# shanjiayao/PTT

Measured on AMD Instinct MI355X. Metric: tracklet frames/sec (hot path: PointNet++ SA stack + Point-Track-Transformer blocks), higher is better.
Workload: dtype f32

## Files before the change

include/ptt_hip.h:

```cpp
#ifndef PTT_HIP_H
#define PTT_HIP_H

#include <stddef.h>
#include <stdint.h>

#ifdef __cplusplus
extern "C" {
#endif

#define PTT_ABI_VERSION 34

enum {
    PTT_OK = 0,
    PTT_EINVAL = -1,
    PTT_EUNSUPPORTED = -2,
    PTT_ELAUNCH = -3,
    PTT_EWORKSPACE = -4
};

typedef void* ptt_stream_t;

int ptt_version(void);
const char* ptt_error_name(int code);
const char* ptt_last_error_string(void);

int ptt_fps_f32(const float* xyz, int B, int N, int npoint, int32_t* idx_out,
                ptt_stream_t stream);
int ptt_fps_ws_f32(const float* xyz, int B, int N, int npoint, int32_t* idx_out, float* workspace,
                   size_t workspace_elems, ptt_stream_t stream);

int ptt_ffps_f32(const float* xyz, const float* feat, int64_t feat_sb, int64_t feat_sc, int64_t feat_sn,
                 int B, int N, int C, int npoint, int32_t* idx_out, ptt_stream_t stream);

int ptt_gather_f32(const float* feat, const int32_t* idx, int B, int C, int N, int M,
                   float* out, ptt_stream_t stream);
int ptt_gather_grad_f32(const float* grad_out, const int32_t* idx, int B, int C, int N,
                        int M, float* grad_feat, ptt_stream_t stream);

int ptt_select_centres_f32(const float* xyz, const int32_t* idx, int B, int N, int M, float* new_xyz,
                           int64_t* idx64_out, ptt_stream_t stream);

int ptt_ball_query_f32(const float* new_xyz, const float* xyz, int B, int M, int N,
                       float radius, int nsample, int32_t* idx_out, ptt_stream_t stream);

int ptt_centres_ball_query_f32(const float* xyz, const int32_t* sel, int B, int N, int M, float radius, int nsample,
                               float* new_xyz, int64_t* idx64_out, int32_t* idx_out, ptt_stream_t stream);

int ptt_group_f32(const float* feat, const int32_t* idx, int B, int C, int N, int M,
                  int ns, float* out, ptt_stream_t stream);
int ptt_group_grad_f32(const float* grad_out, const int32_t* idx, int B, int C, int N,
                       int M, int ns, float* grad_feat, ptt_stream_t stream);

size_t ptt_scatter_add_det_workspace(int B, int N, int E);
int ptt_scatter_add_det_f32(const float* src, const int32_t* idx, int B, int C, int N, int E, float* out,
                            void* workspace, size_t workspace_bytes, ptt_stream_t stream);

int ptt_knn_f32(const float* xyz, int B, int N, int k, int32_t* idx_out,
                ptt_stream_t stream);
int ptt_knn_rel_f32(const float* xyz, int B, int N, int k, int32_t* idx_out, float* rel_out,
                    ptt_stream_t stream);

size_t ptt_packed_weight_elems(int Cout, int K);
// ... 523 lines not shown
```

ptt_amd/csrc/point_ops.hip:

```cpp
#pragma clang fp contract(off)

#include <limits.h>
#include <stdlib.h>
#include "common.h"

namespace ptt {

__device__ __forceinline__ float sqdist3(float ax, float ay, float az, float bx, float by, float bz) {
    const float dx = ax - bx, dy = ay - by, dz = az - bz;
    return (dx * dx + dy * dy) + dz * dz;
}

__device__ __forceinline__ float knn_dist(float ax, float ay, float az, float bx, float by, float bz) {
    const float d = sqdist3(ax, ay, az, bx, by, bz);
    return d < __builtin_inff() ? d : 3.402823466e+38f;
}

__device__ __forceinline__ float lane_bcast(float v, int src_lane) {
    return __builtin_bit_cast(float, __builtin_amdgcn_readlane(__builtin_bit_cast(int, v), src_lane));
}

typedef float fps_f2 __attribute__((ext_vector_type(2)));


// ... 160 lines not shown
            } else if constexpr (LX) {
                lx = xyz_lds[3 * gi + 0]; ly = xyz_lds[3 * gi + 1]; lz = xyz_lds[3 * gi + 2];
            } else {
                if (gd < 0.f) { gx = pts[0]; gy = pts[1]; gz = pts[2]; }
                lx = gx; ly = gy; lz = gz;
            }
            if (t == 0) sel_lds[j] = gi;
        }
    }
    __syncthreads();
    for (int j = t; j < npoint; j += T) out[j] = sel_lds[j];
}

template <int T, int P>
static int launch_fps(const float* xyz, int B, int N, int npoint, int32_t* idx, hipStream_t s) {
    const size_t sel_bytes = (size_t)((npoint + 3) & ~3) * sizeof(int);
    if (sel_bytes + (size_t)N * 12 + 1024 <= 65536 && !dev_switches().fps_plain) {
#ifdef PTT_DEV
        if (const char* e = getenv("PTT_FPS_ABL")) {
            const int abl = atoi(e);
#define PTT_FPS_ABL_CASE(A) if (abl == A) { hipLaunchKernelGGL((fps_kernel<T, P, true, A>), dim3(B), dim3(T), sel_bytes + (size_t)N * 12, s, xyz, N, npoint, idx); return check_launch("fps_kernel(abl)"); }
            PTT_FPS_ABL_CASE(1) PTT_FPS_ABL_CASE(2) PTT_FPS_ABL_CASE(3) PTT_FPS_ABL_CASE(4) PTT_FPS_ABL_CASE(8) PTT_FPS_ABL_CASE(12) PTT_FPS_ABL_CASE(15)
            PTT_FPS_ABL_CASE(16) PTT_FPS_ABL_CASE(32) PTT_FPS_ABL_CASE(47) PTT_FPS_ABL_CASE(7) PTT_FPS_ABL_CASE(24) PTT_FPS_ABL_CASE(40)
#undef PTT_FPS_ABL_CASE
        }
#endif
        hipLaunchKernelGGL((fps_kernel<T, P, true>), dim3(B), dim3(T), sel_bytes + (size_t)N * 12, s, xyz, N, npoint, idx);
        return check_launch("fps_kernel");
    }
    hipLaunchKernelGGL((fps_kernel<T, P, false>), dim3(B), dim3(T), sel_bytes, s, xyz, N, npoint, idx);
    return check_launch("fps_kernel");
}

template <int CPW>
__device__ __forceinline__ void ball_sweep(const float* __restrict__ pts, int N, float r2, int ns, const float (&cx)[CPW],
                                           const float (&cy)[CPW], const float (&cz)[CPW], int ncentres,
                                           int32_t* __restrict__ out0, int lane) {
    int cnt[CPW], first[CPW];
#pragma unroll
    for (int c = 0; c < CPW; ++c) { cnt[c] = (c < ncentres) ? 0 : ns; first[c] = 0; }
    for (int base = 0; base < N; base += 64) {
        const int k = base + lane;
        const bool in = k < N;
        float px = 0.f, py = 0.f, pz = 0.f;
        if (in) { px = pts[3 * k + 0]; py = pts[3 * k + 1]; pz = pts[3 * k + 2]; }
        bool active = false;
#pragma unroll
        for (int c = 0; c < CPW; ++c) {
            if (cnt[c] >= ns) continue;
            const float d = sqdist3(cx[c], cy[c], cz[c], px, py, pz);
            const bool hit = in && d < r2;
            const unsigned long long mask = __ballot(hit);
            if (mask != 0ull) {
                if (cnt[c] == 0) first[c] = base + (__ffsll((long long)mask) - 1);
                const int pos = cnt[c] + __popcll(mask & ((1ull << lane) - 1ull));
                if (hit && pos < ns) out0[(size_t)c * ns + pos] = k;
                cnt[c] += __popcll(mask);
            }
            active = active || cnt[c] < ns;
        }
        if (!active) break;
    }
#pragma unroll
    for (int c = 0; c < CPW; ++c) {
        if (c >= ncentres) break;
        const int fill = (cnt[c] > 0) ? first[c] : 0;
// ... 908 lines not shown
    if (N <= 64) return launch_fps<64, 1>(xyz, B, N, npoint, idx_out, s);
    if (N <= 128) return launch_fps<64, 2>(xyz, B, N, npoint, idx_out, s);
    if (N <= 256) return launch_fps<64, 4>(xyz, B, N, npoint, idx_out, s);
    if (N <= 512) {
        if (const int T = dev_switches().fps_t) {
            if (T == 256) return launch_fps<256, 2>(xyz, B, N, npoint, idx_out, s);
            if (T == 128) return launch_fps<128, 4>(xyz, B, N, npoint, idx_out, s);
            if (T == 512) return launch_fps<512, 1>(xyz, B, N, npoint, idx_out, s);
        }
        return launch_fps<64, 8>(xyz, B, N, npoint, idx_out, s);
    }
    if (N <= 1024) {
        if (const int T = dev_switches().fps_t) {
            if (T == 64) return launch_fps<64, 16>(xyz, B, N, npoint, idx_out, s);
            if (T == 128) return launch_fps<128, 8>(xyz, B, N, npoint, idx_out, s);
            if (T == 512) return launch_fps<512, 2>(xyz, B, N, npoint, idx_out, s);
        }
        return launch_fps<256, 4>(xyz, B, N, npoint, idx_out, s);
    }
    if (N <= 2048) {
        if (const int T = dev_switches().fps_t) {
            if (T == 512) return launch_fps<512, 4>(xyz, B, N, npoint, idx_out, s);
            if (T == 1024) return launch_fps<1024, 2>(xyz, B, N, npoint, idx_out, s);
            if (T == 128) return launch_fps<128, 16>(xyz, B, N, npoint, idx_out, s);
        }
        return launch_fps<256, 8>(xyz, B, N, npoint, idx_out, s);
    }
    if (N <= 4096) return launch_fps<512, 8>(xyz, B, N, npoint, idx_out, s);
    if (N <= 8192) return launch_fps<1024, 8>(xyz, B, N, npoint, idx_out, s);
    if (N <= 16384) return launch_fps<1024, 16>(xyz, B, N, npoint, idx_out, s);
    return fail(PTT_EUNSUPPORTED, "ptt_fps_f32: N=%d exceeds the register-resident limit 16384 (use ptt_fps_ws_f32)", N);
}

extern "C" int ptt_spatial_order_f32(const float* xyz, int B, int N, int32_t* order, ptt_stream_t stream) {
    if (B < 0 || N <= 0) return fail(PTT_EINVAL, "ptt_spatial_order_f32: B=%d N=%d", B, N);
    if (B == 0) return PTT_OK;
    if (!xyz || !order) return fail(PTT_EINVAL, "ptt_spatial_order_f32: null pointer");
    if (N > 8192 || (long long)B * N > INT_MAX) return fail(PTT_EUNSUPPORTED, "ptt_spatial_order_f32: N=%d (at most 8192 points per cloud are sorted in LDS)", N);
    int P = 2;
    while (P < N) P <<= 1;
    const int lds = P * (int)sizeof(unsigned long long);
    return launch("spatial_order_kernel", spatial_order_kernel, dim3(B), dim3(1024), lds, as_stream(stream), xyz, N, P, order);
}

extern "C" int ptt_fps_ws_f32(const float* xyz, int B, int N, int npoint, int32_t* idx_out, float* workspace, size_t workspace_elems,
                              ptt_stream_t stream) {
    if (B < 0 || N <= 0 || npoint < 0) return fail(PTT_EINVAL, "ptt_fps_ws_f32: B=%d N=%d npoint=%d", B, N, npoint);
    if (B == 0 || npoint == 0) return PTT_OK;
    if (!xyz || !idx_out) return fail(PTT_EINVAL, "ptt_fps_ws_f32: null pointer");
    if ((long long)N * 3 > INT_MAX) return fail(PTT_EUNSUPPORTED, "ptt_fps_ws_f32: N=%d", N);
    if (!workspace || workspace_elems < (size_t)B * N)
        return fail(PTT_EWORKSPACE, "ptt_fps_ws_f32: %zu floats of workspace needed", (size_t)B * N);
    hipLaunchKernelGGL(fps_ws_kernel, dim3(B), dim3(1024), 0, as_stream(stream), xyz, N, npoint, workspace, idx_out);
    return check_launch("fps_ws_kernel");
}

extern "C" int ptt_ffps_f32(const float* xyz, const float* feat, int64_t feat_sb, int64_t feat_sc, int64_t feat_sn, int B, int N, int C,
                            int npoint, int32_t* idx_out, ptt_stream_t stream) {
    if (B < 1 || N < 1 || npoint < 1 || C < 0) return fail(PTT_EINVAL, "ptt_ffps_f32: B=%d N=%d C=%d npoint=%d", B, N, C, npoint);
    if (!xyz || !idx_out || (C > 0 && !feat)) return fail(PTT_EINVAL, "ptt_ffps_f32: null pointer");
    if (N > FFPS_MAX_N || C > FFPS_MAX_C || npoint > FFPS_MAX_NPOINT)
        return fail(PTT_EUNSUPPORTED, "ptt_ffps_f32: N=%d C=%d npoint=%d exceed the limits N <= %d, C <= %d, npoint <= %d", N, C, npoint,
                    FFPS_MAX_N, FFPS_MAX_C, FFPS_MAX_NPOINT);
    if (C > 0 && (long long)(N - 1) * llabs((long long)feat_sn) + (long long)(C - 1) * llabs((long long)feat_sc) > INT_MAX)
        return fail(PTT_EUNSUPPORTED, "ptt_ffps_f32: one cloud's features span more than 2^31 elements (strides %lld, %lld)",
                    (long long)feat_sc, (long long)feat_sn);
// ... 292 lines not shown
```

ptt_amd/models/backbones_3d/pointnet2/pointnet2_modules.py:

```python
import os
from typing import List

import torch
import torch.nn as nn
import torch.nn.functional as F

from .... import ops, train_ops
from ....param_cache import (DropsCachesOnModeChange, FoldedLayer, ParamCache, conv_bn_tensors, fold_conv_bn,
                             index_table)
from . import pointnet2_utils
from . import pytorch_utils as pt_utils

STREAM_COMPACT_MIN_BALLS = 2048
STREAM_COMPACT_MAX_POINTS = 1024


class PointnetSAModuleVotes(DropsCachesOnModeChange, nn.Module):
    def __init__(self, *, mlp: List[int], radius: float = None, nsample: int = None, bn: bool = True,
                 use_xyz: bool = True, normalize_xyz: bool = False, sample_uniformly: bool = False,
                 sample_method='fps'):
        super().__init__()
        self.radius = radius
        self.nsample = nsample
        self.mlp_module = None
        self.use_xyz = use_xyz
        self.normalize_xyz = normalize_xyz
        self.sample_uniformly = sample_uniformly
        self.grouper = pointnet2_utils.QueryAndGroup(radius, nsample, use_xyz=use_xyz, ret_grouped_xyz=True,
                                                     normalize_xyz=normalize_xyz, sample_uniformly=sample_uniformly,
                                                     ret_unique_cnt=False)
        mlp_spec = mlp
        if use_xyz and len(mlp_spec) > 0:
            mlp_spec[0] += 3
        self.mlp_module = pt_utils.SharedMLP(mlp_spec, bn=bn)
        self.sample_method = sample_method
        self._fused_cache = ParamCache()
        self.centres_knn_k = 0
        self.centres_knn = None

    def _sample(self, xyz, features, npoint):
        if self.sample_method == 'fps':
            return pointnet2_utils.furthest_point_sample(xyz, npoint)
        if self.sample_method in ('rs', 'sequence'):
            return index_table(xyz.size(0), npoint, xyz.device, torch.int32)
        if self.sample_method == 'ffps':
            if features is None:
                raise ValueError("sample_method 'ffps': a level without point features cannot sample in feature space "
                                 "(use 'fps' for it)")
            return ops.feature_fps(xyz.contiguous(), features.detach(), npoint)
        raise NotImplementedError(self.sample_method)

    def _fusable(self, xyz, features):
        if self.training or not xyz.is_cuda:
            return False
        name = 'PointnetSAModuleVotes(nsample=%s, mlp=%s)' % (self.nsample, [u.conv.weight.shape[0] for u in self.mlp_module
                                                                              if hasattr(u, 'conv')])
        if ops.autograd_recording(self, xyz, features):
            return ops.note_unfused(name, 'autograd is recording (wrap inference in torch.no_grad())')
        if self.sample_uniformly or self.nsample not in (16, 32, 64):
            return ops.note_unfused(name, 'nsample must be 16, 32 or 64 and sample_uniformly off')
        if xyz.dtype != torch.float32 or (features is not None and features.dtype != torch.float32):
            return ops.note_unfused(name, 'inputs must be float32')
        if len(self.mlp_module) > 4:
            return ops.note_unfused(name, 'more than 4 SharedMLP layers')
        for unit in self.mlp_module:
            conv = getattr(unit, 'conv', None)
            if conv is None or conv.kernel_size != (1, 1) or conv.weight.shape[0] % 32 != 0 or conv.weight.shape[0] > 256:
                return ops.note_unfused(name, 'layer widths must be multiples of 32, at most 256, 1x1 convolutions')
            if list(unit._modules.keys())[0] != 'conv':
                return ops.note_unfused(name, 'pre-activation units')
        return True

    def _fused_params(self, device):
        return self._fused_cache.get(conv_bn_tensors(self.mlp_module), device, self._fold)
# ... 104 lines not shown
```

ptt_amd/models/backbones_3d/pointnet2/pointnet2_utils.py:

```python
import torch
import torch.nn as nn
from torch.autograd import Function

from .... import ops


class _FurthestPointSampling(Function):
    @staticmethod
    def forward(ctx, xyz, npoint):
        return ops.furthest_point_sampling(xyz.contiguous(), npoint)

    @staticmethod
    def backward(ctx, grad=None):
        return None, None


class _GatherOperation(Function):
    @staticmethod
    def forward(ctx, features, idx):
        ctx.n = features.shape[2]
        ctx.save_for_backward(idx)
        return ops.gather_points(features.contiguous(), idx.contiguous())

    @staticmethod
    def backward(ctx, grad_out):
        (idx,) = ctx.saved_tensors
        return ops.gather_points_grad(grad_out.contiguous(), idx, ctx.n), None


class _GroupingOperation(Function):
    @staticmethod
    def forward(ctx, features, idx):
        ctx.n = features.shape[2]
        ctx.save_for_backward(idx)
        return ops.group_points(features.contiguous(), idx.contiguous())

    @staticmethod
    def backward(ctx, grad_out):
        (idx,) = ctx.saved_tensors
        return ops.group_points_grad(grad_out.contiguous(), idx, ctx.n), None


class _BallQuery(Function):
    @staticmethod
    def forward(ctx, radius, nsample, xyz, new_xyz):
        return ops.ball_query(new_xyz.contiguous(), xyz.contiguous(), radius, nsample)

    @staticmethod
    def backward(ctx, grad=None):
        return None, None, None, None


def _not_reached(name):
    def fn(*args, **kwargs):
        raise NotImplementedError(
            "%s: defined by the reference wrappers but never called anywhere in PTT; not provided" % name)
    return fn


furthest_point_sample = _FurthestPointSampling.apply
gather_operation = _GatherOperation.apply
grouping_operation = _GroupingOperation.apply
ball_query = _BallQuery.apply
furthest_point_sampling_with_dist = _not_reached("furthest_point_sampling_with_dist")
three_nn = _not_reached("three_nn")
three_interpolate = _not_reached("three_interpolate")


class QueryAndGroup(nn.Module):

    def __init__(self, radius, nsample, use_xyz=True, ret_grouped_xyz=False, normalize_xyz=False,
                 sample_uniformly=False, ret_unique_cnt=False):
        super().__init__()
        self.radius, self.nsample, self.use_xyz = radius, nsample, use_xyz
        self.ret_grouped_xyz = ret_grouped_xyz
        self.normalize_xyz = normalize_xyz
        self.sample_uniformly = sample_uniformly
        self.ret_unique_cnt = ret_unique_cnt
        if ret_unique_cnt:
            assert sample_uniformly

    def _resample_uniformly(self, idx):
        unique_cnt = torch.zeros((idx.shape[0], idx.shape[1]))
        for b in range(idx.shape[0]):
            for r in range(idx.shape[1]):
                uniq = torch.unique(idx[b, r, :])
                n = uniq.shape[0]
                unique_cnt[b, r] = n
                pick = torch.randint(0, n, (self.nsample - n,), dtype=torch.long, device=uniq.device)
                idx[b, r, :] = torch.cat((uniq, uniq[pick]))
        return idx, unique_cnt

    def forward(self, xyz, new_xyz, features=None, return_idx=False):
# ... 45 lines not shown
```

ptt_amd/models/backbones_3d/pointnet2_backbone.py:

```python
from typing import List

import torch
import torch.nn as nn

from ... import graph_policy, ops, train_ops
from ...param_cache import ParamCache, index_table
from .pointnet2 import pointnet2_modules


class PointNet2BackboneLight(nn.Module):
    def __init__(self, model_cfg, input_channels, **kwargs):
        super().__init__()
        self.model_cfg = model_cfg
        input_channels -= 3
        self.num_points_each_layer = []
        self.SA_modules = nn.ModuleList()
        sa = self.model_cfg.SA_CONFIG
        for k in range(len(sa.RADIUS)):
            mlps = list(sa.MLPS[k])
            if k == 0:
                mlps[0] = input_channels
            self.SA_modules.append(pointnet2_modules.PointnetSAModuleVotes(
                radius=sa.RADIUS[k], nsample=sa.NSAMPLE[k], mlp=mlps,
                use_xyz=sa.get('USE_XYZ', True), normalize_xyz=sa.get('NORMALIZE_XYZ', True),
# ... 11 lines not shown
        features = pc[..., 3:].contiguous() if pc.size(-1) > 3 else None
        return xyz, features

    def _cov_final(self, features):
        if not features.is_cuda:
            return self.cov_final(features)
        if self.training:
            if features.dtype != torch.float32:
                return self.cov_final(features)
            return train_ops.rows_linear(self.cov_final, features.transpose(1, 2)).transpose(1, 2)
        if ops.autograd_recording(self.cov_final, features) or features.dtype != torch.float32:
            ops.note_unfused('PointNet2BackboneLight.cov_final', 'autograd is recording or input is not float32')
            return self.cov_final(features)
        w, b = self.cov_final.weight, self.cov_final.bias
        wpacked, bias = self._cov_cache.get([w, b], w.device, lambda: (ops.pack_weight(w), b.detach().float().contiguous()))
        rows = features.transpose(1, 2)
        out = ops.linear(rows, wpacked, w.shape[0], None, bias)
        return out.transpose(1, 2)

    def branch_forward(self, pts, npoints: List, inds0=None, want_knn=0, compact_levels=()):
        xyz, features = self._break_up_pc(pts)
        sa = self.model_cfg.SA_CONFIG
        one_frame = (not self.training and xyz.is_cuda and features is None and len(self.SA_modules) == 3
                     and xyz.shape[0] * npoints[0] <= 4 * ops.ONE_FRAME_MAX_POINTS
                     and self.SA_modules[0].sample_method == 'fps'
                     and all(m.sample_method in ('rs', 'sequence') for m in self.SA_modules[1:])
                     and npoints[0] >= npoints[1] >= npoints[2] and (not want_knn or npoints[2] <= 128)
                     and all(m._fusable(xyz, None) for m in self.SA_modules[:1]))
        knn = None
        if one_frame:
            from .pointnet2 import pointnet2_utils
            xyz = xyz.contiguous()
            if inds0 is None:
                inds0 = pointnet2_utils.furthest_point_sample(xyz, npoints[0])
            inds0 = inds0.to(torch.int32).contiguous()
            levels, inds64, knn = ops.sa_levels_point_jobs(xyz, inds0, list(npoints), list(sa.RADIUS), list(sa.NSAMPLE),
                                                           knn_k=want_knn)
            seq = [None] + [index_table(xyz.size(0), n, xyz.device, torch.int64) for n in npoints[1:3]]
            xyz, features, inds0 = self.SA_modules[0](xyz=xyz, features=features, npoint=npoints[0], inds=inds0,
                                                      pre=(levels[0][0], levels[0][1], inds64))
            xyz, features, inds1 = self.SA_modules[1](xyz=xyz, features=features, npoint=npoints[1],
                                                      pre=(levels[1][0], levels[1][1], seq[1]))
            xyz, features, inds2 = self.SA_modules[2](xyz=xyz, features=features, npoint=npoints[2],
                                                      pre=(levels[2][0], levels[2][1], seq[2]))
        else:
            xyz, features, inds0 = self.SA_modules[0](xyz=xyz, features=features, npoint=npoints[0], inds=inds0)
            xyz, features, inds1 = self.SA_modules[1](xyz=xyz, features=features, npoint=npoints[1], compact=1 in compact_levels)
            xyz, features, inds2 = self.SA_modules[2](xyz=xyz, features=features, npoint=npoints[2], compact=2 in compact_levels)
        point_features = self._cov_final(features)
        assert inds1.dtype == inds2.dtype == torch.int64, 'index type must be int64, not {}'.format(inds2.dtype)
        if all(m.sample_method in ('rs', 'sequence') for m in self.SA_modules[1:]) and inds0.shape[1] >= npoints[2]:
            inds = inds0[:, :npoints[2]]
        else:
            inds = inds0.gather(1, inds1).gather(1, inds2)
        if want_knn:
            return xyz, point_features, inds, knn
        return xyz, point_features, inds

    def sample(self, search_points, template_points):
        from .pointnet2 import pointnet2_utils
        sa = self.model_cfg.SA_CONFIG
        assert sa.SAMPLE_METHOD[0] == 'fps'
        return (pointnet2_utils.furthest_point_sample(search_points[..., 0:3].contiguous(), sa.NPOINTS_SEARCH[0]),
                pointnet2_utils.furthest_point_sample(template_points[..., 0:3].contiguous(), sa.NPOINTS_TEMPLATE[0]))

    def forward_branches(self, search_points, template_points, inds=None):
        sa = self.model_cfg.SA_CONFIG
# ... 32 lines not shown
```

ptt_amd/ops.py:

```python
import contextlib
import ctypes
import math
import os

import torch

from . import _lib
from ._lib import AttnDesc, SaDesc, SaLayer, XcorrDesc


def _stream():
    return ctypes.c_void_p(torch.cuda.current_stream().cuda_stream)


_timing = None


def start_kernel_timing(names):
    global _timing
    _timing = {n: [] for n in names}


def stop_kernel_timing():
    global _timing
# ... 93 lines not shown
    return t


def _ptr(t):
    return ctypes.c_void_p(t.data_ptr()) if t is not None else ctypes.c_void_p(0)


_UNTIMED = contextlib.nullcontext()


def _launch(name, device, *args, timed=None):
    with torch.cuda.device(device), (_timed(timed) if timed else _UNTIMED):
        rc = getattr(_lib.lib(), name)(*args, _stream())
    if rc:
        _lib.check(rc, name)


def _host(name, *args):
    return getattr(_lib.lib(), name)(*args)


def _host_checked(name, *args):
    _lib.check(_host(name, *args), name)


def _workspace(query, device, *dims):
    ws = _ws(_host(query, *dims), device)
    return ws, (_ptr(ws), ws.numel() * 8)


FPS_RESIDENT_MAX_N, FPS_RESIDENT_MAX_NPOINT = 16384, 15360


def furthest_point_sampling(xyz, npoint):
    _chk(xyz, "xyz", torch.float32, 3)
    B, N, _ = xyz.shape
    out = torch.empty((B, int(npoint)), dtype=torch.int32, device=xyz.device)
    if N <= FPS_RESIDENT_MAX_N and int(npoint) <= FPS_RESIDENT_MAX_NPOINT:
        _launch("ptt_fps_f32", xyz.device, _ptr(xyz), B, N, int(npoint), _ptr(out), timed='ptt_fps_f32')
    else:
        ws = torch.empty((B * N,), dtype=torch.float32, device=xyz.device)
        _launch("ptt_fps_ws_f32", xyz.device, _ptr(xyz), B, N, int(npoint), _ptr(out), _ptr(ws), ws.numel(), timed='ptt_fps_f32')
    return out


FFPS_MAX_N, FFPS_MAX_C, FFPS_MAX_NPOINT = 16384, 1024, 15360


def feature_fps(xyz, features, npoint):
    _chk(xyz, "xyz", torch.float32, 3)
    B, N, _ = xyz.shape
    C = 0
    if features is not None:
        if not isinstance(features, torch.Tensor):
            raise TypeError("features must be a torch.Tensor")
        if not features.is_cuda:
            raise RuntimeError("features must be a device (HIP) tensor — CPU tensors are not supported")
        if features.dtype != torch.float32:
            raise RuntimeError("features must be torch.float32, got %s" % features.dtype)
        if features.dim() != 3 or features.shape[0] != B or features.shape[2] != N:
            raise RuntimeError("features must be (B,C,N) = (%d,C,%d), got %s" % (B, N, tuple(features.shape)))
        C = features.shape[1]
    npoint = int(npoint)
    if N > FFPS_MAX_N or C > FFPS_MAX_C or npoint > FFPS_MAX_NPOINT:
        raise ValueError("feature_fps: N=%d, C=%d, npoint=%d exceed the kernel's limits N <= %d, C <= %d, npoint <= %d"
                         % (N, C, npoint, FFPS_MAX_N, FFPS_MAX_C, FFPS_MAX_NPOINT))
    if N < 1 or npoint < 1:
        raise ValueError("feature_fps: N=%d and npoint=%d must be at least 1" % (N, npoint))
    out = torch.empty((B, npoint), dtype=torch.int32, device=xyz.device)
    if B == 0:
        return out
    sb, sc, sn = features.stride() if C else (0, 0, 0)
    if C and (N - 1) * abs(sn) + (C - 1) * abs(sc) > 2 ** 31 - 1:
        raise ValueError("feature_fps: one cloud's features span more than 2^31 - 1 elements (strides %d, %d)" % (sc, sn))
    _launch("ptt_ffps_f32", xyz.device, _ptr(xyz), _ptr(features if C else None), sb, sc, sn, B, N, C, npoint, _ptr(out),
# ... 1773 lines not shown
```

Baseline: 17380.

## Deduplicate coincident points before furthest point sampling and run FPS on unique set

Adds a distinct-point FPS kernel. It builds an LDS hash table to collapse identical xyz points, keeping the lowest index of each, then compacts the unique indices. The serial FPS chain then runs over only the unique points: in a single wave with no block barriers when the unique count is small, otherwise across the block. The first-level SA sampling without features and the backbone's initial FPS are switched to this path. The aim is to cut the per-iteration serial FPS cost on resampled clouds that contain many duplicate points. The cost is hashing and atomics up front, plus possible tie-break and tail-fill differences once all remaining distances reach zero.

New measurement: 17430 (median of 6 runs). Within noise of the previous version (+0.3%).

```diff
diff --git a/include/ptt_hip.h b/include/ptt_hip.h
--- a/include/ptt_hip.h
+++ b/include/ptt_hip.h
@@ -8,7 +8,7 @@
 extern "C" {
 #endif
 
-#define PTT_ABI_VERSION 34
+#define PTT_ABI_VERSION 35
 
 enum {
     PTT_OK = 0,
@@ -28,6 +28,7 @@
                 ptt_stream_t stream);
 int ptt_fps_ws_f32(const float* xyz, int B, int N, int npoint, int32_t* idx_out, float* workspace,
                    size_t workspace_elems, ptt_stream_t stream);
+int ptt_fps_distinct_f32(const float* xyz, int B, int N, int npoint, int32_t* idx_out, ptt_stream_t stream);
 
 int ptt_ffps_f32(const float* xyz, const float* feat, int64_t feat_sb, int64_t feat_sc, int64_t feat_sn,
                  int B, int N, int C, int npoint, int32_t* idx_out, ptt_stream_t stream);
diff --git a/ptt_amd/csrc/point_ops.hip b/ptt_amd/csrc/point_ops.hip
--- a/ptt_amd/csrc/point_ops.hip
+++ b/ptt_amd/csrc/point_ops.hip
@@ -216,6 +216,241 @@
     return check_launch("fps_kernel");
 }
 
+constexpr int FPSD_T = 256, FPSD_W = FPSD_T / 64, FPSD_EMPTY = INT_MAX;
+constexpr int FPSD_PW = 12;
+
+__device__ __forceinline__ unsigned fpsd_bits(float v) {
+    return v == 0.f ? 0u : __builtin_bit_cast(unsigned, v);
+}
+
+template <int Q>
+__device__ __forceinline__ void fpsd_load(const float* xyz_lds, const int* cidx, int U, int p0, float (&px)[Q], float (&py)[Q],
+                                          float (&pz)[Q], float (&md)[Q], int (&oi)[Q]) {
+#pragma unroll
+    for (int i = 0; i < Q; ++i) {
+        float x = 0.f, y = 0.f, z = 0.f, m = -1.0f;
+        int o = 0;
+        if (p0 + i < U) {
+            o = cidx[p0 + i];
+            x = xyz_lds[3 * o + 0]; y = xyz_lds[3 * o + 1]; z = xyz_lds[3 * o + 2];
+            const float mag = (x * x + y * y) + z * z;
+            m = (mag > 1e-3f) ? 1e10f : -1.0f;
+        }
+        px[i] = x; py[i] = y; pz[i] = z; md[i] = m; oi[i] = o;
+    }
+}
+
+template <int Q>
+__device__ __forceinline__ void fpsd_scan(const float (&px)[Q], const float (&py)[Q], const float (&pz)[Q], float (&md)[Q],
+                                          const int (&oi)[Q], float lx, float ly, float lz, float& best, int& besti) {
+    static_assert(Q % 2 == 0, "two points at a time");
+    best = -1.0f; besti = 0;
+    const fps_f2 lxv = {lx, lx}, lyv = {ly, ly}, lzv = {lz, lz};
+#pragma unroll
+    for (int i = 0; i < Q; i += 2) {
+        const fps_f2 dx = fps_f2{px[i], px[i + 1]} - lxv, dy = fps_f2{py[i], py[i + 1]} - lyv, dz = fps_f2{pz[i], pz[i + 1]} - lzv;
+        const fps_f2 d = (dx * dx + dy * dy) + dz * dz;
+#pragma unroll
+        for (int h = 0; h < 2; ++h) {
+            const float m = fminf(md[i + h], d[h]);
+            md[i + h] = m;
+            const bool take = m > best;
+            best = take ? m : best;
+            besti = take ? oi[i + h] : besti;
+        }
+    }
+}
+
+template <int Q>
+__device__ __forceinline__ void fpsd_chain_wave(const float* xyz_lds, const int* cidx, int U, int npoint, int* sel, int lane) {
+    float px[Q], py[Q], pz[Q], md[Q];
+    int oi[Q];
+    fpsd_load<Q>(xyz_lds, cidx, U, lane * Q, px, py, pz, md, oi);
+    float lx = xyz_lds[0], ly = xyz_lds[1], lz = xyz_lds[2];
+    int j = 1, widx = 0;
+    bool more = npoint > 1;
+    while (more) {
+        float best;
+        int besti;
+        fpsd_scan<Q>(px, py, pz, md, oi, lx, ly, lz, best, besti);
+        const float wmax = wave_max_f32_fused(best);
+        const int src = __ffsll((long long)__ballot(best == wmax)) - 1;
+        widx = __builtin_amdgcn_readlane(besti, src);
+        if (wmax < 0.f) widx = 0;
+        const float* w = xyz_lds + __umul24(widx, 3);
+        lx = w[0]; ly = w[1]; lz = w[2];
+        if (lane == 0) sel[j] = widx;
+        ++j;
+        more = (wmax > 0.f) & (j < npoint);
+    }
+    for (int jj = j + lane; jj < npoint; jj += 64) sel[jj] = widx;
+}
+
+template <int P>
+__device__ __forceinline__ void fpsd_chain_group(const float* xyz_lds, const int* cidx, int U, int npoint, int* sel,
+                                                 float2 (*slots)[FPSD_W], int t) {
+    const int lane = t & 63, wv = t >> 6;
+    float px[P], py[P], pz[P], md[P];
+    int oi[P];
+    fpsd_load<P>(xyz_lds, cidx, U, t * P, px, py, pz, md, oi);
+    float lx = xyz_lds[0], ly = xyz_lds[1], lz = xyz_lds[2];
+    int j = 1, gi = 0;
+    bool more = npoint > 1;
+    while (more) {
+        float best;
+        int besti;
+        fpsd_scan<P>(px, py, pz, md, oi, lx, ly, lz, best, besti);
+        const float wmax = wave_max_f32_fused(best);
+        const int src = __ffsll((long long)__ballot(best == wmax)) - 1;
+        const int par = j & 1;
+        if (lane == src) slots[par][wv] = make_float2(best, __builtin_bit_cast(float, besti));
+        __syncthreads();
+        float gd = -1.0f;
+        gi = 0;
+#pragma unroll
+        for (int w = 0; w < FPSD_W; ++w) {
+            const float2 s2 = slots[par][w];
+            const bool take = s2.x > gd;
+            gd = take ? s2.x : gd;
+            gi = take ? __builtin_bit_cast(int, s2.y) : gi;
+        }
+        if (gd < 0.f) gi = 0;
+        const float* w = xyz_lds + __umul24(gi, 3);
+        lx = w[0]; ly = w[1]; lz = w[2];
+        if (t == 0) sel[j] = gi;
+        ++j;
+        more = (gd > 0.f) & (j < npoint);
+    }
+    for (int jj = j + t; jj < npoint; jj += FPSD_T) sel[jj] = gi;
+}
+
+template <int P, int PW>
+__global__ __launch_bounds__(FPSD_T) void fps_distinct_kernel(const float* __restrict__ xyz, int N, int npoint, int M, int shift,
+                                                              int32_t* __restrict__ idx_out) {
+    static_assert(P * FPSD_W <= 64, "the chunk counts are scanned by one wave");
+    const int b = blockIdx.x, t = threadIdx.x, lane = t & 63, wv = t >> 6;
+    const float* __restrict__ pts = xyz + (size_t)b * N * 3;
+    int32_t* __restrict__ out = idx_out + (size_t)b * npoint;
+
+    extern __shared__ int fpsd_lds[];
+    int* sel = fpsd_lds;
+    float* xyz_lds = reinterpret_cast<float*>(fpsd_lds + ((npoint + 3) & ~3));
+    int* table = reinterpret_cast<int*>(xyz_lds + 3 * N);
+    __shared__ int chunk_cnt[P * FPSD_W];
+    __shared__ float2 slots[2][FPSD_W];
+
+    float x[P], y[P], z[P];
+#pragma unroll
+    for (int r = 0; r < P; ++r) {
+        const int k = r * FPSD_T + t;
+        x[r] = y[r] = z[r] = 0.f;
+        if (k < N) {
+            x[r] = pts[3 * k + 0]; y[r] = pts[3 * k + 1]; z[r] = pts[3 * k + 2];
+            xyz_lds[3 * k + 0] = x[r]; xyz_lds[3 * k + 1] = y[r]; xyz_lds[3 * k + 2] = z[r];
+        }
+    }
+    for (int h = t; h < M; h += FPSD_T) table[h] = FPSD_EMPTY;
+    if (t == 0 && npoint > 0) sel[0] = 0;
+    __syncthreads();
+
+    int slot[P], cur[P];
+#pragma unroll
+    for (int r = 0; r < P; ++r) {
+        const int k = r * FPSD_T + t;
+        slot[r] = 0; cur[r] = FPSD_EMPTY;
+        if (k < N) {
+            unsigned h = fpsd_bits(x[r]) * 0x9E3779B1u ^ fpsd_bits(y[r]) * 0x85EBCA77u ^ fpsd_bits(z[r]) * 0xC2B2AE3Du;
+            h = ((h ^ (h >> 15)) * 0x2C1B3C6Du) >> shift;
+            slot[r] = (int)h;
+            cur[r] = atomicCAS(&table[h], FPSD_EMPTY, k);
+        }
+    }
+    bool same[P];
+#pragma unroll
+    for (int r = 0; r < P; ++r) {
+        same[r] = false;
+        if (cur[r] != FPSD_EMPTY) {
+            const float* o = xyz_lds + __umul24(cur[r], 3);
+            same[r] = o[0] == x[r] && o[1] == y[r] && o[2] == z[r];
+        }
+    }
+#pragma unroll
+    for (int r = 0; r < P; ++r) {
+        const int k = r * FPSD_T + t;
+        if (same[r]) {
+            atomicMin(&table[slot[r]], k);
+        } else if (cur[r] != FPSD_EMPTY) {
+            unsigned h = (unsigned)slot[r];
+            for (;;) {
+                h = (h + 1) & (unsigned)(M - 1);
+                const int c = atomicCAS(&table[h], FPSD_EMPTY, k);
+                if (c == FPSD_EMPTY) break;
+                const float* o = xyz_lds + __umul24(c, 3);
+                if (o[0] == x[r] && o[1] == y[r] && o[2] == z[r]) {
+                    atomicMin(&table[h], k);
+                    break;
+                }
+            }
+            slot[r] = (int)h;
+        }
+    }
+    __syncthreads();
+
+    unsigned long long keep[P];
+#pragma unroll
+    for (int r = 0; r < P; ++r) {
+        const int k = r * FPSD_T + t;
+        keep[r] = __ballot(k < N && table[slot[r]] == k);
+        if (lane == 0) chunk_cnt[r * FPSD_W + wv] = __popcll(keep[r]);
+    }
+    __syncthreads();
+    const int cnt = lane < P * FPSD_W ? chunk_cnt[lane] : 0;
+    int incl = cnt;
+#pragma unroll
+    for (int off = 1; off < 64; off <<= 1) {
+        const int v = __shfl_up(incl, off, 64);
+        if (lane >= off) incl += v;
+    }
+    const int U = __builtin_amdgcn_readlane(incl, 63);
+    const int excl = incl - cnt;
+    int* cidx = table;
+#pragma unroll
+    for (int r = 0; r < P; ++r) {
+        const int base = __builtin_amdgcn_readlane(excl, r * FPSD_W + wv);
+        if ((keep[r] >> lane) & 1ull) cidx[base + __popcll(keep[r] & ((1ull << lane) - 1ull))] = r * FPSD_T + t;
+    }
+    __syncthreads();
+
+    if (U <= 64 * PW) {
+        if (wv == 0) {
+            if (U <= 128) fpsd_chain_wave<2>(xyz_lds, cidx, U, npoint, sel, lane);
+            else if (U <= 256) fpsd_chain_wave<4>(xyz_lds, cidx, U, npoint, sel, lane);
+            else if (U <= 384) fpsd_chain_wave<6>(xyz_lds, cidx, U, npoint, sel, lane);
+            else if (PW > 8 && U <= 512) fpsd_chain_wave<8>(xyz_lds, cidx, U, npoint, sel, lane);
+            else if (PW > 10 && U <= 640) fpsd_chain_wave<10>(xyz_lds, cidx, U, npoint, sel, lane);
+            else fpsd_chain_wave<PW>(xyz_lds, cidx, U, npoint, sel, lane);
+        }
+    } else if constexpr (FPSD_T * P > 64 * PW) {
+        if (P > 4 && U <= FPSD_T * 4) fpsd_chain_group<4>(xyz_lds, cidx, U, npoint, sel, slots, t);
+        else fpsd_chain_group<P>(xyz_lds, cidx, U, npoint, sel, slots, t);
+    }
+    __syncthreads();
+    for (int j = t; j < npoint; j += FPSD_T) out[j] = sel[j];
+}
+
+template <int P>
+static int launch_fps_distinct(const float* xyz, int B, int N, int npoint, int M, int lds, int32_t* idx, hipStream_t s) {
+    int shift = 32;
+    while ((1 << (32 - shift)) < M) --shift;
+#ifdef PTT_DEV
+    if (const char* e = getenv("PTT_FPSD_PW")) {
+        if (atoi(e) == 8) return launch("fps_distinct_kernel(C=512)", fps_distinct_kernel<P, 8>, dim3(B), dim3(FPSD_T), lds, s, xyz, N, npoint, M, shift, idx);
+        if (atoi(e) == 10) return launch("fps_distinct_kernel(C=640)", fps_distinct_kernel<P, 10>, dim3(B), dim3(FPSD_T), lds, s, xyz, N, npoint, M, shift, idx);
+    }
+#endif
+    return launch("fps_distinct_kernel", fps_distinct_kernel<P, FPSD_PW>, dim3(B), dim3(FPSD_T), lds, s, xyz, N, npoint, M, shift, idx);
+}
+
 template <int CPW>
 __device__ __forceinline__ void ball_sweep(const float* __restrict__ pts, int N, float r2, int ns, const float (&cx)[CPW],
                                            const float (&cy)[CPW], const float (&cz)[CPW], int ncentres,
@@ -1190,6 +1425,20 @@
     return fail(PTT_EUNSUPPORTED, "ptt_fps_f32: N=%d exceeds the register-resident limit 16384 (use ptt_fps_ws_f32)", N);
 }
 
+extern "C" int ptt_fps_distinct_f32(const float* xyz, int B, int N, int npoint, int32_t* idx_out, ptt_stream_t stream) {
+    if (B < 0 || N <= 0 || npoint < 0) return fail(PTT_EINVAL, "ptt_fps_distinct_f32: B=%d N=%d npoint=%d", B, N, npoint);
+    if (B == 0 || npoint == 0) return PTT_OK;
+    if (!xyz || !idx_out) return fail(PTT_EINVAL, "ptt_fps_distinct_f32: null pointer");
+    int M = 256;
+    while (M < 2 * N && M < (1 << 20)) M <<= 1;
+    const size_t lds = (size_t)((npoint + 3) & ~3) * sizeof(int) + (size_t)N * 12 + (size_t)M * sizeof(int);
+    if (N <= 64 || N > 2048 || lds + 1024 > 65536) return ptt_fps_f32(xyz, B, N, npoint, idx_out, stream);
+    hipStream_t s = as_stream(stream);
+    if (N <= 512) return launch_fps_distinct<2>(xyz, B, N, npoint, M, (int)lds, idx_out, s);
+    if (N <= 1024) return launch_fps_distinct<4>(xyz, B, N, npoint, M, (int)lds, idx_out, s);
+    return launch_fps_distinct<8>(xyz, B, N, npoint, M, (int)lds, idx_out, s);
+}
+
 extern "C" int ptt_spatial_order_f32(const float* xyz, int B, int N, int32_t* order, ptt_stream_t stream) {
     if (B < 0 || N <= 0) return fail(PTT_EINVAL, "ptt_spatial_order_f32: B=%d N=%d", B, N);
     if (B == 0) return PTT_OK;
diff --git a/ptt_amd/models/backbones_3d/pointnet2/pointnet2_modules.py b/ptt_amd/models/backbones_3d/pointnet2/pointnet2_modules.py
--- a/ptt_amd/models/backbones_3d/pointnet2/pointnet2_modules.py
+++ b/ptt_amd/models/backbones_3d/pointnet2/pointnet2_modules.py
@@ -40,6 +40,8 @@
 
     def _sample(self, xyz, features, npoint):
         if self.sample_method == 'fps':
+            if features is None:
+                return pointnet2_utils.furthest_point_sample_distinct(xyz, npoint)
             return pointnet2_utils.furthest_point_sample(xyz, npoint)
         if self.sample_method in ('rs', 'sequence'):
             return index_table(xyz.size(0), npoint, xyz.device, torch.int32)
diff --git a/ptt_amd/models/backbones_3d/pointnet2/pointnet2_utils.py b/ptt_amd/models/backbones_3d/pointnet2/pointnet2_utils.py
--- a/ptt_amd/models/backbones_3d/pointnet2/pointnet2_utils.py
+++ b/ptt_amd/models/backbones_3d/pointnet2/pointnet2_utils.py
@@ -9,6 +9,17 @@
     @staticmethod
     def forward(ctx, xyz, npoint):
         return ops.furthest_point_sampling(xyz.contiguous(), npoint)
+
+    @staticmethod
+    def backward(ctx, grad=None):
+        return None, None
+
+
+class _FurthestPointSamplingDistinct(Function):
+
+    @staticmethod
+    def forward(ctx, xyz, npoint):
+        return ops.furthest_point_sampling_distinct(xyz.contiguous(), npoint)
 
     @staticmethod
     def backward(ctx, grad=None):
@@ -59,6 +70,7 @@
 
 
 furthest_point_sample = _FurthestPointSampling.apply
+furthest_point_sample_distinct = _FurthestPointSamplingDistinct.apply
 gather_operation = _GatherOperation.apply
 grouping_operation = _GroupingOperation.apply
 ball_query = _BallQuery.apply
diff --git a/ptt_amd/models/backbones_3d/pointnet2_backbone.py b/ptt_amd/models/backbones_3d/pointnet2_backbone.py
--- a/ptt_amd/models/backbones_3d/pointnet2_backbone.py
+++ b/ptt_amd/models/backbones_3d/pointnet2_backbone.py
@@ -67,7 +67,7 @@
             from .pointnet2 import pointnet2_utils
             xyz = xyz.contiguous()
             if inds0 is None:
-                inds0 = pointnet2_utils.furthest_point_sample(xyz, npoints[0])
+                inds0 = pointnet2_utils.furthest_point_sample_distinct(xyz, npoints[0])
             inds0 = inds0.to(torch.int32).contiguous()
             levels, inds64, knn = ops.sa_levels_point_jobs(xyz, inds0, list(npoints), list(sa.RADIUS), list(sa.NSAMPLE),
                                                            knn_k=want_knn)
diff --git a/ptt_amd/ops.py b/ptt_amd/ops.py
--- a/ptt_amd/ops.py
+++ b/ptt_amd/ops.py
@@ -158,6 +158,20 @@
     else:
         ws = torch.empty((B * N,), dtype=torch.float32, device=xyz.device)
         _launch("ptt_fps_ws_f32", xyz.device, _ptr(xyz), B, N, int(npoint), _ptr(out), _ptr(ws), ws.numel(), timed='ptt_fps_f32')
+    return out
+
+
+FPS_DISTINCT = True
+
+
+def furthest_point_sampling_distinct(xyz, npoint):
+    if not (FPS_DISTINCT and isinstance(xyz, torch.Tensor) and xyz.is_cuda and xyz.dim() == 3
+            and xyz.shape[1] <= FPS_RESIDENT_MAX_N and int(npoint) <= FPS_RESIDENT_MAX_NPOINT):
+        return furthest_point_sampling(xyz, npoint)
+    _chk(xyz, "xyz", torch.float32, 3)
+    B, N, _ = xyz.shape
+    out = torch.empty((B, int(npoint)), dtype=torch.int32, device=xyz.device)
+    _launch("ptt_fps_distinct_f32", xyz.device, _ptr(xyz), B, N, int(npoint), _ptr(out), timed='ptt_fps_f32')
     return out
 
 
```

## Add deduplicating FPS kernel that runs the sampling chain on distinct points

Applied to the files above, without the earlier changes.

Adds a new FPS kernel that hashes point coordinates in LDS to find duplicate points. When the distinct count fits in one wave's capacity, it compacts them and runs the serial FPS chain on a single 64-lane wave, with no block-wide barriers per iteration. It also exits early once the max distance reaches zero and fills the remaining indices. The first-level FPS on raw point clouds is routed to this kernel, trading hash-table setup cost and a risk of differing tie-breaking for a cheaper sequential loop on padded or duplicated inputs.

Result: no change. 17400 before, 17320 after (-0.4%).

```diff
diff --git a/include/ptt_hip.h b/include/ptt_hip.h
--- a/include/ptt_hip.h
+++ b/include/ptt_hip.h
@@ -8,7 +8,7 @@
 extern "C" {
 #endif
 
-#define PTT_ABI_VERSION 34
+#define PTT_ABI_VERSION 35
 
 enum {
     PTT_OK = 0,
@@ -28,6 +28,10 @@
                 ptt_stream_t stream);
 int ptt_fps_ws_f32(const float* xyz, int B, int N, int npoint, int32_t* idx_out, float* workspace,
                    size_t workspace_elems, ptt_stream_t stream);
+#define PTT_FPS_DISTINCT_MAX_N 2048
+#define PTT_FPS_DISTINCT_CAPACITY 640
+int ptt_fps_distinct_f32(const float* xyz, int B, int N, int npoint, int32_t* idx_out,
+                         ptt_stream_t stream);
 
 int ptt_ffps_f32(const float* xyz, const float* feat, int64_t feat_sb, int64_t feat_sc, int64_t feat_sn,
                  int B, int N, int C, int npoint, int32_t* idx_out, ptt_stream_t stream);
diff --git a/ptt_amd/csrc/point_ops.hip b/ptt_amd/csrc/point_ops.hip
--- a/ptt_amd/csrc/point_ops.hip
+++ b/ptt_amd/csrc/point_ops.hip
@@ -216,6 +216,174 @@
     return check_launch("fps_kernel");
 }
 
+constexpr int FPSD_PS = 10;
+constexpr int FPSD_CAP = 64 * FPSD_PS;
+constexpr int FPSD_EMPTY = 0x7fffffff;
+static_assert(FPSD_CAP == PTT_FPS_DISTINCT_CAPACITY, "ptt_hip.h states the one-wave capacity");
+
+template <int T, int P>
+__device__ __forceinline__ void fpsd_chain(const float* cx, int n, int npoint, int t, int* sel, float (*slots)[T / 64][2], int* fin) {
+    static_assert(P % 2 == 0, "packed update");
+    constexpr int W = T / 64;
+    const int lane = t & 63, wv = t >> 6;
+    float px[P], py[P], pz[P], md[P];
+#pragma unroll
+    for (int i = 0; i < P; ++i) {
+        const int k = t * P + i;
+        float x = 0.f, y = 0.f, z = 0.f, m = -1.0f;
+        if (k < n) {
+            x = cx[3 * k + 0]; y = cx[3 * k + 1]; z = cx[3 * k + 2];
+            const float mag = (x * x + y * y) + z * z;
+            m = (mag > 1e-3f) ? 1e10f : -1.0f;
+        }
+        px[i] = x; py[i] = y; pz[i] = z; md[i] = m;
+    }
+    float lx = cx[0], ly = cx[1], lz = cx[2];
+    for (int j = 1; j < npoint; ++j) {
+        float best = -1.0f;
+        int besti = 0;
+        const fps_f2 lxv = {lx, lx}, lyv = {ly, ly}, lzv = {lz, lz};
+#pragma unroll
+        for (int i = 0; i < P; i += 2) {
+            const fps_f2 dx = fps_f2{px[i], px[i + 1]} - lxv, dy = fps_f2{py[i], py[i + 1]} - lyv, dz = fps_f2{pz[i], pz[i + 1]} - lzv;
+            const fps_f2 d = (dx * dx + dy * dy) + dz * dz;
+#pragma unroll
+            for (int h = 0; h < 2; ++h) {
+                const float m = fminf(md[i + h], d[h]);
+                md[i + h] = m;
+                const bool take = m > best;
+                best = take ? m : best;
+                besti = take ? t * P + i + h : besti;
+            }
+        }
+        const float wmax = wave_max_f32_fused(best);
+        const int src = __ffsll((long long)__ballot(best == wmax)) - 1;
+        float gd;
+        int gi;
+        if constexpr (W == 1) {
+            gd = wmax;
+            gi = __builtin_amdgcn_readlane(besti, src);
+        } else {
+            const int par = j & 1;
+            if (lane == src) *reinterpret_cast<float2*>(slots[par][wv]) = make_float2(best, __builtin_bit_cast(float, besti));
+            __syncthreads();
+            float fd = -1.0f;
+            int fi = 0;
+#pragma unroll
+            for (int w = 0; w < W; ++w) {
+                const float2 s2 = *reinterpret_cast<const float2*>(slots[par][w]);
+                const bool take = s2.x > fd;
+                fd = take ? s2.x : fd;
+                fi = take ? __builtin_bit_cast(int, s2.y) : fi;
+            }
+            gd = fd; gi = fi;
+        }
+        if (gd < 0.f) gi = 0;
+        lx = cx[3 * gi + 0]; ly = cx[3 * gi + 1]; lz = cx[3 * gi + 2];
+        if (t == 0) sel[j] = gi;
+        if (__builtin_amdgcn_readfirstlane(__builtin_bit_cast(int, gd)) <= 0) {
+            if (t == 0) { fin[0] = j; fin[1] = gi; }
+            break;
+        }
+    }
+}
+
+template <int T, int P>
+__global__ __launch_bounds__(T) void fps_distinct_kernel(const float* __restrict__ xyz, int N, int npoint, int32_t* __restrict__ idx_out) {
+    constexpr int W = T / 64, CAPN = T * P, H = W > 1 ? 2 * CAPN : 1024;
+    const int b = blockIdx.x, t = threadIdx.x;
+    const float* __restrict__ pts = xyz + (size_t)b * N * 3;
+    int32_t* __restrict__ out = idx_out + (size_t)b * npoint;
+
+    __shared__ __attribute__((aligned(16))) float xyz_lds[3 * CAPN];
+    __shared__ int tab[H];
+    __shared__ __attribute__((aligned(16))) float slots[2][W][2];
+    __shared__ int fin[2];
+    __shared__ unsigned short list[W > 1 ? CAPN : 2];
+    __shared__ unsigned short slot_of[W > 1 ? CAPN : 2];
+    __shared__ __attribute__((aligned(16))) float cxyz[W > 1 ? 3 * FPSD_CAP : 4];
+    __shared__ int wtot[W];
+
+    for (int e = t; e < 3 * N; e += T) xyz_lds[e] = pts[e];
+    if (t == 0) { fin[0] = npoint; fin[1] = 0; }
+    bool mapped = false;
+    if constexpr (W == 1) {
+        if (t == 0) tab[0] = 0;
+        __syncthreads();
+        fpsd_chain<64, P>(xyz_lds, N, npoint, t, tab, slots, fin);
+    } else {
+        for (int e = t; e < H; e += T) tab[e] = FPSD_EMPTY;
+        __syncthreads();
+        const unsigned* ux = reinterpret_cast<const unsigned*>(xyz_lds);
+#pragma unroll 1
+        for (int k = t; k < N; k += T) {
+            const unsigned a = ux[3 * k + 0], c = ux[3 * k + 1], d = ux[3 * k + 2];
+            unsigned h = (a * 0x9E3779B1u) ^ (c * 0x85EBCA77u) ^ (d * 0xC2B2AE3Du);
+            h ^= h >> 15; h *= 0x2C1B3C6Du; h ^= h >> 13;
+            int s = (int)(h & (unsigned)(H - 1));
+            for (;;) {
+                const int cur = atomicCAS(&tab[s], FPSD_EMPTY, k);
+                if (cur == FPSD_EMPTY) break;
+                if (ux[3 * cur + 0] == a && ux[3 * cur + 1] == c && ux[3 * cur + 2] == d) {
+                    if (k < cur) atomicMin(&tab[s], k);
+                    break;
+                }
+                s = (s + 1) & (H - 1);
+            }
+            slot_of[k] = (unsigned short)s;
+        }
+        __syncthreads();
+        unsigned firsts = 0;
+#pragma unroll
+        for (int i = 0; i < P; ++i) {
+            const int k = t * P + i;
+            if (k < N && tab[slot_of[k]] == k) firsts |= 1u << i;
+        }
+        const int cnt = __popc(firsts), lane = t & 63, wv = t >> 6;
+        int incl = cnt;
+#pragma unroll
+        for (int off = 1; off < 64; off <<= 1) {
+            const int v = __shfl_up(incl, off, 64);
+            if (lane >= off) incl += v;
+        }
+        if (lane == 63) wtot[wv] = incl;
+        __syncthreads();
+        int pos = incl - cnt, U = 0;
+#pragma unroll
+        for (int w = 0; w < W; ++w) {
+            const int s = wtot[w];
+            pos += w < wv ? s : 0;
+            U += s;
+        }
+        if (t == 0) tab[0] = 0;
+        if (U <= FPSD_CAP) {
+            mapped = true;
+#pragma unroll
+            for (int i = 0; i < P; ++i) {
+                if (firsts >> i & 1u) {
+                    const int k = t * P + i;
+                    list[pos] = (unsigned short)k;
+                    cxyz[3 * pos + 0] = xyz_lds[3 * k + 0]; cxyz[3 * pos + 1] = xyz_lds[3 * k + 1]; cxyz[3 * pos + 2] = xyz_lds[3 * k + 2];
+                    ++pos;
+                }
+            }
+            __syncthreads();
+            if (wv == 0) fpsd_chain<64, FPSD_PS>(cxyz, U, npoint, t, tab, nullptr, fin);
+        } else {
+            fpsd_chain<T, P>(xyz_lds, N, npoint, t, tab, slots, fin);
+        }
+    }
+    __syncthreads();
+    const int rounds = fin[0], fill = mapped ? (int)list[fin[1]] : fin[1];
+    for (int j = t; j < npoint; j += T) out[j] = j >= rounds ? fill : mapped ? (int)list[tab[j]] : tab[j];
+}
+
+template <int T, int P>
+static int launch_fps_distinct(const float* xyz, int B, int N, int npoint, int32_t* idx, hipStream_t s) {
+    hipLaunchKernelGGL((fps_distinct_kernel<T, P>), dim3(B), dim3(T), 0, s, xyz, N, npoint, idx);
+    return check_launch("fps_distinct_kernel");
+}
+
 template <int CPW>
 __device__ __forceinline__ void ball_sweep(const float* __restrict__ pts, int N, float r2, int ns, const float (&cx)[CPW],
                                            const float (&cy)[CPW], const float (&cz)[CPW], int ncentres,
@@ -1190,6 +1358,18 @@
     return fail(PTT_EUNSUPPORTED, "ptt_fps_f32: N=%d exceeds the register-resident limit 16384 (use ptt_fps_ws_f32)", N);
 }
 
+extern "C" int ptt_fps_distinct_f32(const float* xyz, int B, int N, int npoint, int32_t* idx_out, ptt_stream_t stream) {
+    if (B < 0 || N <= 0 || npoint < 0) return fail(PTT_EINVAL, "ptt_fps_distinct_f32: B=%d N=%d npoint=%d", B, N, npoint);
+    if (B == 0 || npoint == 0) return PTT_OK;
+    if (!xyz || !idx_out) return fail(PTT_EINVAL, "ptt_fps_distinct_f32: null pointer");
+    hipStream_t s = as_stream(stream);
+    if (N <= 256 && npoint <= 1024) return launch_fps_distinct<64, 4>(xyz, B, N, npoint, idx_out, s);
+    if (N <= 512 && npoint <= 1024) return launch_fps_distinct<64, 8>(xyz, B, N, npoint, idx_out, s);
+    if (N > 512 && N <= 1024 && npoint <= 2048) return launch_fps_distinct<256, 4>(xyz, B, N, npoint, idx_out, s);
+    if (N > 1024 && N <= PTT_FPS_DISTINCT_MAX_N && npoint <= 4096) return launch_fps_distinct<256, 8>(xyz, B, N, npoint, idx_out, s);
+    return ptt_fps_f32(xyz, B, N, npoint, idx_out, stream);
+}
+
 extern "C" int ptt_spatial_order_f32(const float* xyz, int B, int N, int32_t* order, ptt_stream_t stream) {
     if (B < 0 || N <= 0) return fail(PTT_EINVAL, "ptt_spatial_order_f32: B=%d N=%d", B, N);
     if (B == 0) return PTT_OK;
diff --git a/ptt_amd/models/backbones_3d/pointnet2/pointnet2_modules.py b/ptt_amd/models/backbones_3d/pointnet2/pointnet2_modules.py
--- a/ptt_amd/models/backbones_3d/pointnet2/pointnet2_modules.py
+++ b/ptt_amd/models/backbones_3d/pointnet2/pointnet2_modules.py
@@ -40,6 +40,8 @@
 
     def _sample(self, xyz, features, npoint):
         if self.sample_method == 'fps':
+            if features is None:
+                return pointnet2_utils.furthest_point_sample_inline(xyz, npoint)
             return pointnet2_utils.furthest_point_sample(xyz, npoint)
         if self.sample_method in ('rs', 'sequence'):
             return index_table(xyz.size(0), npoint, xyz.device, torch.int32)
diff --git a/ptt_amd/models/backbones_3d/pointnet2/pointnet2_utils.py b/ptt_amd/models/backbones_3d/pointnet2/pointnet2_utils.py
--- a/ptt_amd/models/backbones_3d/pointnet2/pointnet2_utils.py
+++ b/ptt_amd/models/backbones_3d/pointnet2/pointnet2_utils.py
@@ -59,6 +59,14 @@
 
 
 furthest_point_sample = _FurthestPointSampling.apply
+
+
+def furthest_point_sample_inline(xyz, npoint):
+    if xyz.is_cuda:
+        return ops.furthest_point_sampling(xyz.contiguous(), npoint, distinct=True)
+    return furthest_point_sample(xyz, npoint)
+
+
 gather_operation = _GatherOperation.apply
 grouping_operation = _GroupingOperation.apply
 ball_query = _BallQuery.apply
diff --git a/ptt_amd/models/backbones_3d/pointnet2_backbone.py b/ptt_amd/models/backbones_3d/pointnet2_backbone.py
--- a/ptt_amd/models/backbones_3d/pointnet2_backbone.py
+++ b/ptt_amd/models/backbones_3d/pointnet2_backbone.py
@@ -67,7 +67,7 @@
             from .pointnet2 import pointnet2_utils
             xyz = xyz.contiguous()
             if inds0 is None:
-                inds0 = pointnet2_utils.furthest_point_sample(xyz, npoints[0])
+                inds0 = pointnet2_utils.furthest_point_sample_inline(xyz, npoints[0])
             inds0 = inds0.to(torch.int32).contiguous()
             levels, inds64, knn = ops.sa_levels_point_jobs(xyz, inds0, list(npoints), list(sa.RADIUS), list(sa.NSAMPLE),
                                                            knn_k=want_knn)
diff --git a/ptt_amd/ops.py b/ptt_amd/ops.py
--- a/ptt_amd/ops.py
+++ b/ptt_amd/ops.py
@@ -149,11 +149,17 @@
 FPS_RESIDENT_MAX_N, FPS_RESIDENT_MAX_NPOINT = 16384, 15360
 
 
-def furthest_point_sampling(xyz, npoint):
+FPS_DISTINCT = True
+FPS_DISTINCT_MAX_N = _lib.DEFINES["PTT_FPS_DISTINCT_MAX_N"]
+
+
+def furthest_point_sampling(xyz, npoint, distinct=False):
     _chk(xyz, "xyz", torch.float32, 3)
     B, N, _ = xyz.shape
     out = torch.empty((B, int(npoint)), dtype=torch.int32, device=xyz.device)
-    if N <= FPS_RESIDENT_MAX_N and int(npoint) <= FPS_RESIDENT_MAX_NPOINT:
+    if distinct and FPS_DISTINCT and N <= FPS_DISTINCT_MAX_N and int(npoint) <= FPS_RESIDENT_MAX_NPOINT:
+        _launch("ptt_fps_distinct_f32", xyz.device, _ptr(xyz), B, N, int(npoint), _ptr(out), timed='ptt_fps_f32')
+    elif N <= FPS_RESIDENT_MAX_N and int(npoint) <= FPS_RESIDENT_MAX_NPOINT:
         _launch("ptt_fps_f32", xyz.device, _ptr(xyz), B, N, int(npoint), _ptr(out), timed='ptt_fps_f32')
     else:
         ws = torch.empty((B * N,), dtype=torch.float32, device=xyz.device)
```
